# denix56/SI-Mamba

Hardware: AMD Instinct MI355X
Metric: point-clouds/sec (fwd+bwd) (higher is better)
Workload: dtype f32; 1 GPU; PointMamba classifier train step (FPS+kNN grouping, encoder, spectral SAST ordering, 12 Mamba blocks d=384 at L=1024, head, AdamW), 1024 pts -> 128 patches; global_batch=64, per_gpu_batch=64, npoints=1024, patches=128, mamba_seq_len=1024, parallelism=dp1, communicator_ranks=1, library_gemm=tuned solution table (si_mamba_amd/tuned/gemm_gfx950.csv)

## Files before the change

si_mamba_amd/csrc/mfma_device.h:

```cpp
#pragma once
#include <type_traits>

#include "common.h"

namespace simamba {

typedef float f32x16 __attribute__((ext_vector_type(16)));
typedef float f32x4 __attribute__((ext_vector_type(4)));
typedef unsigned u32x4 __attribute__((ext_vector_type(4)));
typedef __bf16 bf16x8 __attribute__((ext_vector_type(8)));

using rsrc_t = __amdgpu_buffer_rsrc_t;
constexpr unsigned kOob = 0xfffff000u;

__device__ __forceinline__ rsrc_t make_rsrc(const void* base, unsigned bytes) {
  return __builtin_amdgcn_make_buffer_rsrc(const_cast<void*>(base), 0, static_cast<int>(bytes), 0x00020000);
}
using bvec4_t = decltype(__builtin_amdgcn_raw_buffer_load_b128(make_rsrc(nullptr, 0u), 0u, 0u, 0));
template <typename V>
__device__ __forceinline__ V bload16(rsrc_t r, unsigned voff, unsigned soff) {
  return __builtin_bit_cast(V, __builtin_amdgcn_raw_buffer_load_b128(r, voff, soff, 0));
}
template <typename V>
__device__ __forceinline__ void bstore16(V v, rsrc_t r, unsigned voff, unsigned soff) {
  __builtin_amdgcn_raw_buffer_store_b128(__builtin_bit_cast(bvec4_t, v), r, voff, soff, 0);
}
__device__ __forceinline__ void bstore4(float f, rsrc_t r, unsigned voff, unsigned soff) {
  __builtin_amdgcn_raw_buffer_store_b32(__builtin_bit_cast(unsigned, f), r, voff, soff, 0);
}
__device__ __forceinline__ void bstore2(unsigned short v, rsrc_t r, unsigned voff, unsigned soff) {
  __builtin_amdgcn_raw_buffer_store_b16(v, r, voff, soff, 0);
}

template <int I, int N, typename F>
__device__ __forceinline__ void static_for(F&& f) {
  if constexpr (I < N) {
    f(std::integral_constant<int, I>{});
    static_for<I + 1, N>(f);
  }
}
template <int OFF, typename V>
__device__ __forceinline__ void lds_read16(V& dst, unsigned addr) {
  asm volatile("ds_read_b128 %0, %1 offset:%2" : "=v"(dst) : "v"(addr), "n"(OFF) : "memory");
}
template <int N, typename V>
__device__ __forceinline__ void lds_wait(V& v) {
  asm volatile("s_waitcnt lgkmcnt(%1)" : "+v"(v) : "n"(N) : "memory");
}

__device__ __forceinline__ unsigned bf16_pack2(float lo, float hi) {
  return static_cast<unsigned>(f32_to_bf16(lo)) | (static_cast<unsigned>(f32_to_bf16(hi)) << 16);
}
__device__ __forceinline__ float bf16_lo(unsigned w) { return __builtin_bit_cast(float, w << 16); }
__device__ __forceinline__ float bf16_hi(unsigned w) { return __builtin_bit_cast(float, w & 0xffff0000u); }

}
```

si_mamba_amd/csrc/scan_bwd_seq.hip:

```cpp
#include "scan_host.h"
#include "scan_seq_common.h"
#include "scan_xlane.h"

namespace simamba {

#ifndef SIMAMBA_BWDSEQ_OCC
#define SIMAMBA_BWDSEQ_OCC 3
#endif
constexpr int kBsSeg = 16;
constexpr int kBsR = 16;
constexpr int kBsWaves = 4;
constexpr int kBsThreads = 64 * kBsWaves;
constexpr int kBsCh = kBsR * kBsWaves;
constexpr int kBsTile = kBsR * kSeqTC;
constexpr int kBsPPitch = 33;
constexpr int kBsWaveFloats = 4 * kBsTile + kSeqTC * kBsPPitch;
constexpr int kBsSmemFloats = kBsWaves * kBsWaveFloats + kSeqTC * 32;

struct BwdSeqArgs {
  const void* u; const void* delta; const void* z; const void* dout;
  void* du; void* ddelta; void* dz;
  const float* A; const float* D; const float* delta_bias;
  const void* B; const void* C;
  const void* dt; const void* wdt;
  long long dt_bs, dt_ts;
  int dt_rank;
  const float* ckpt;
  float* dA; float* dB; float* dC; float* dD; float* ddelta_bias;
  int batch, dim, seqlen, nck;
  int bc_mode;
  long long z_bs, dz_bs;
  long long bc_bs, bc_ns, bc_ts;
};

__device__ __forceinline__ float bs_row_finish(float w0, float w1) {
  float d;
  asm("s_nop 1\n\t"
      "v_add_f32_dpp %0, %1, %1 row_ror:8 row_mask:0xf bank_mask:0x3\n\t"
      "v_add_f32_dpp %0, %2, %2 row_ror:8 row_mask:0xf bank_mask:0xc\n\t"
      "s_nop 1\n\t"
      "v_add_f32_dpp %0, %0, %0 row_shr:4 row_mask:0xf bank_mask:0xa"
      : "=&v"(d)
      : "v"(w0), "v"(w1));
  return d;
}

__device__ __forceinline__ void bs_quad_sum1(float& a) {
  asm("s_nop 1\n\t"
      "v_add_f32_dpp %0, %0, %0 quad_perm:[1,0,3,2] row_mask:0xf bank_mask:0xf\n\t"
      "s_nop 1\n\t"
      "v_add_f32_dpp %0, %0, %0 quad_perm:[2,3,0,1] row_mask:0xf bank_mask:0xf"
      : "+v"(a));
}
__device__ __forceinline__ void bs_quad_sum2(float& a, float& b) {
  asm("s_nop 1\n\t"
      "v_add_f32_dpp %0, %0, %0 quad_perm:[1,0,3,2] row_mask:0xf bank_mask:0xf\n\t"
      "v_add_f32_dpp %1, %1, %1 quad_perm:[1,0,3,2] row_mask:0xf bank_mask:0xf\n\t"
      "s_nop 0\n\t"
      "v_add_f32_dpp %0, %0, %0 quad_perm:[2,3,0,1] row_mask:0xf bank_mask:0xf\n\t"
      "v_add_f32_dpp %1, %1, %1 quad_perm:[2,3,0,1] row_mask:0xf bank_mask:0xf"
      : "+v"(a), "+v"(b));
}

template <typename T, bool kHasZ, bool kDt = false, bool kDet = false>
__global__ __launch_bounds__(kBsThreads, SIMAMBA_BWDSEQ_OCC) void scan_bwd_seq_kernel(BwdSeqArgs p) {
  __shared__ __attribute__((aligned(16))) float smem[kBsSmemFloats];
  const int tid = threadIdx.x;
  const int lane = tid & 63;
  const int wave = __builtin_amdgcn_readfirstlane(tid >> 6);
  int tile_id, b;
  xcd_tile(tile_id, b);
  const int L = p.seqlen, D = p.dim;
  const int d0w = tile_id * kBsCh + wave * kBsR;
  float* tD = smem + wave * kBsWaveFloats;
  float* tU = tD + kBsTile;
  float* tY = tU + kBsTile;
  float* tZ = tY + kBsTile;
  float* tP = tZ + kBsTile;
  float* tBC = smem + kBsWaves * kBsWaveFloats;

  const int r4 = lane >> 4, cq = (lane >> 2) & 3, pq = lane & 3;
  const int ch = 4 * r4 + cq;
  const int dch = d0w + ch;
  float A2[4];
  {
    const float4 a4 = *reinterpret_cast<const float4*>(p.A + static_cast<size_t>(dch) * kMaxState + 4 * pq);
    A2[0] = a4.x * kLog2e; A2[1] = a4.y * kLog2e; A2[2] = a4.z * kLog2e; A2[3] = a4.w * kLog2e;
  }
  const float Dfull = p.D ? p.D[dch] : 0.f;
  float ga[4] = {0.f, 0.f, 0.f, 0.f};
  float dAacc[4] = {0.f, 0.f, 0.f, 0.f};
  float dDacc = 0.f;
  const int sw = (ch >> 1) & 7;
  const int trow = ch * kSeqTC;
  const int pf = (r4 >> 1) * 16 + 4 * pq + 2 * (r4 & 1) + (cq >> 1);
  const float* ckl = p.ckpt + (static_cast<size_t>(b) * p.nck * D + dch) * kMaxState + 4 * pq;
  float* tDb = smem + wave * kBsWaveFloats + 4 * kBsTile + kSeqTC;
  if (kDet && lane < kBsR) tDb[lane * kBsPPitch] = 0.f;

  constexpr unsigned kEsz = sizeof(T);
  const unsigned zdelta = (static_cast<unsigned>(b * p.z_bs) - static_cast<unsigned>(b) * D * L) * kEsz;
  const unsigned dzdelta = (static_cast<unsigned>(b * p.dz_bs) - static_cast<unsigned>(b) * D * L) * kEsz;
  const T* __restrict__ ug = static_cast<const T*>(p.u);
  const T* __restrict__ dg = static_cast<const T*>(p.delta);
  const T* __restrict__ zg = static_cast<const T*>(p.z);
  const T* __restrict__ gg = static_cast<const T*>(p.dout);
  T* __restrict__ dug = static_cast<T*>(p.du);
  T* __restrict__ ddg = static_cast<T*>(p.ddelta);
  T* __restrict__ dzg = static_cast<T*>(p.dz);
  auto lane_now = [&]() -> int {
    int l = __builtin_amdgcn_mbcnt_hi(~0u, __builtin_amdgcn_mbcnt_lo(~0u, 0u));
    asm volatile("" : "+v"(l));
    return l;
  };
  auto row_off = [&](int l, int j) -> unsigned {
    return ((static_cast<unsigned>(b) * D + d0w + (l >> 3) + 8 * j) * L + 4 * (l & 7)) * kEsz;
  };

  const bool tok = p.bc_mode == 2;
  const T* __restrict__ Bgp = static_cast<const T*>(p.B) + static_cast<long long>(b) * p.bc_bs;
  const T* __restrict__ Cgp = static_cast<const T*>(p.C) + static_cast<long long>(b) * p.bc_bs;
  float bcv[4];
  auto issue_bc = [&](int t0, int tv) {
    const bool isC = tok ? (tv & 4) != 0 : (tv >> 7) != 0;
    const int bc_n = tok ? 4 * (tv & 3) : ((tv >> 3) & 15);
    const int bc_tl = tok ? (tv >> 3) : 4 * (tv & 7);
    const int t = (t0 + bc_tl < L) ? t0 + bc_tl : 0;
    const unsigned o = static_cast<unsigned>(bc_n * static_cast<int>(p.bc_ns) + t * static_cast<int>(p.bc_ts)) * kEsz;
    float vb[4], vc[4];
    if (isC) load4<T>(Cgp, o, vc); else load4<T>(Bgp, o, vb);
#pragma unroll
    for (int k = 0; k < 4; ++k) bcv[k] = isC ? vc[k] : vb[k];
  };
  auto stage_bc = [&](int tv) {
    if (tok) {
      *reinterpret_cast<float4*>(tBC + (tv >> 3) * 32 + 4 * (tv & 7)) = make_float4(bcv[0], bcv[1], bcv[2], bcv[3]);
    } else {
      float* dst = tBC + 4 * (tv & 7) * 32 + (tv >> 7) * 16 + ((tv >> 3) & 15);
#pragma unroll
      for (int k = 0; k < 4; ++k) dst[k * 32] = bcv[k];
    }
  };

  float dv[2][4], uv[2][4], gv[2][4], zv[2][4], hsn[4], biasA[2];
  auto form_delta = [&](int t0, int l) {
    const int mc = l & 15, mk = l >> 4;
    const T* wrow = static_cast<const T*>(p.wdt) + static_cast<size_t>(d0w + mc) * p.dt_rank;
    biasA[0] = p.delta_bias ? p.delta_bias[d0w + mc] : 0.f;
#pragma unroll
    for (int tile = 0; tile < 2; ++tile) {
      const int tt = t0 + 16 * tile + mc;
      const T* dtrow = static_cast<const T*>(p.dt) + static_cast<long long>(b) * p.dt_bs +
                       static_cast<long long>(tt < L ? tt : 0) * p.dt_ts;
      f32x4_t acc = {0.f, 0.f, 0.f, 0.f};
      if constexpr (sizeof(T) == 4) {
        const int c0 = (mk & 1) * 4 + (mk >> 1);
        float a[6], w[6];
#pragma unroll
        for (int m = 0; m < 6; ++m) {
          const int r = 8 * (m >> 1) + c0 + 2 * (m & 1);
          const int rc = min(r, p.dt_rank - 1);
          a[m] = reinterpret_cast<const float*>(dtrow)[rc];
          w[m] = reinterpret_cast<const float*>(wrow)[rc];
        }
#pragma unroll
        for (int m = 0; m < 6; ++m) {
          const int r = 8 * (m >> 1) + c0 + 2 * (m & 1);
          acc = __builtin_amdgcn_mfma_f32_16x16x4f32(r < p.dt_rank ? a[m] : 0.f, w[m], acc, 0, 0, 0);
        }
      } else {
        const int kc = min(8 * mk, p.dt_rank - 8);
        uint4 a8 = *reinterpret_cast<const uint4*>(reinterpret_cast<const uint16_t*>(dtrow) + kc);
        const uint4 w8 = *reinterpret_cast<const uint4*>(reinterpret_cast<const uint16_t*>(wrow) + kc);
        if (8 * mk >= p.dt_rank) a8 = make_uint4(0u, 0u, 0u, 0u);
        acc = __builtin_amdgcn_mfma_f32_16x16x32_bf16(__builtin_bit_cast(bf16x8, a8), __builtin_bit_cast(bf16x8, w8),
                                                      acc, 0, 0, 0);
#pragma unroll
        for (int e = 0; e < 4; ++e) acc[e] = bf16_to_f32(f32_to_bf16(acc[e]));
      }
#pragma unroll
      for (int e = 0; e < 4; ++e) dv[tile][e] = acc[e];
    }
  };
  auto load_state = [&](int ts) {
    float4 h4 = make_float4(0.f, 0.f, 0.f, 0.f);
    if (ts > 0 && ts < L) h4 = *reinterpret_cast<const float4*>(ckl + static_cast<size_t>(ts / kBsSeg - 1) * D * kMaxState);
    hsn[0] = h4.x; hsn[1] = h4.y; hsn[2] = h4.z; hsn[3] = h4.w;
  };
  auto issue_loads = [&](int t0, int l) {
    const int qv = l & 7;
    const bool in = t0 + 4 * qv < L;
    const unsigned to = in ? t0 * kEsz : 0u - 4u * qv * kEsz;
#pragma unroll
    for (int j = 0; j < 2; ++j) {
      const unsigned ro = row_off(l, j) + to;
      if (!kDt) load4<T>(dg, ro, dv[j]);
      load4<T>(ug, ro, uv[j]);
      load4<T>(gg, ro, gv[j]);
      if (kHasZ) load4<T>(zg, ro + zdelta, zv[j]);
      if (!kDt) biasA[j] = p.delta_bias ? p.delta_bias[d0w + (l >> 3) + 8 * j] : 0.f;
    }
    if (kDt) form_delta(t0, l);
    load_state(t0 + kBsSeg);
  };

  const int nchunks = (L + kSeqTC - 1) / kSeqTC;
  {
    const int t0 = (nchunks - 1) * kSeqTC;
    const int l = lane_now();
    issue_bc(t0, wave * 64 + l);
    issue_loads(t0, l);
    stage_bc(wave * 64 + l);
  }

  for (int c = nchunks - 1; c >= 0; --c) {
    const int t0 = c * kSeqTC;
    __syncthreads();

    {
      const int l = lane_now();
      const bool in_seq = t0 + 4 * (l & 7) < L;
      if (kDt) {
        const int mc = l & 15, mk = l >> 4;
#pragma unroll
        for (int tile = 0; tile < 2; ++tile) {
          const int qm = 4 * tile + mk;
          const float b2 = (t0 + 4 * qm < L) ? biasA[0] * kLog2e : -1e30f;
          float dl[4];
#pragma unroll
          for (int i = 0; i < 4; ++i) dl[i] = softplus_log2(fmaf(dv[tile][i], kLog2e, b2));
          *reinterpret_cast<float4*>(tD + tile_off(mc, qm)) = make_float4(dl[0], dl[1], dl[2], dl[3]);
        }
      }
#pragma unroll
      for (int j = 0; j < 2; ++j) {
        const float b2 = in_seq ? biasA[j] * kLog2e : -1e30f;
        float dl[4], dyv[4], dzw[4];
#pragma unroll
        for (int i = 0; i < 4; ++i) {
          if (!kDt) dl[i] = softplus_log2(fmaf(dv[j][i], kLog2e, b2));
          const float go = in_seq ? gv[j][i] : 0.f;
          if (kHasZ) {
            const float z = zv[j][i], sg = sigmoid_f(z);
            dyv[i] = go * z * sg;
            dzw[i] = go * sg * (1.f + z * (1.f - sg));
          } else {
            dyv[i] = go;
          }
        }
        const int to_ = tile_off((l >> 3) + 8 * j, l & 7);
        if (!kDt) *reinterpret_cast<float4*>(tD + to_) = make_float4(dl[0], dl[1], dl[2], dl[3]);
        *reinterpret_cast<float4*>(tU + to_) = make_float4(uv[j][0], uv[j][1], uv[j][2], uv[j][3]);
        *reinterpret_cast<float4*>(tY + to_) = make_float4(dyv[0], dyv[1], dyv[2], dyv[3]);
        if (kHasZ) *reinterpret_cast<float4*>(tZ + to_) = make_float4(dzw[0], dzw[1], dzw[2], dzw[3]);
      }
    }
    __builtin_amdgcn_fence(__ATOMIC_RELEASE, "wavefront");
    __builtin_amdgcn_wave_barrier();

#pragma unroll 1
    for (int seg = 1; seg >= 0; --seg) {
      const int ts = t0 + kBsSeg * seg;
      if (ts >= L) { load_state(t0); continue; }
      const float* bcp = tBC + seg * (kBsSeg * 32) + 4 * pq;
      const int gb = 4 * seg;

      float H[kBsSeg][4];
      {
        float h[4] = {hsn[0], hsn[1], hsn[2], hsn[3]};
        float d4[4], u4[4], z4[4];
#ifndef SIMAMBA_BWDSEQ_NOPREFETCH
        float4 b4n = *reinterpret_cast<const float4*>(bcp);
        float4 c4n = *reinterpret_cast<const float4*>(bcp + 16);
#endif
#pragma unroll
        for (int i = 0; i < kBsSeg; ++i) {
          const int o = trow + 4 * ((gb + (i >> 2)) ^ sw);
          if ((i & 3) == 0) {
            const float4 dd = *reinterpret_cast<const float4*>(tD + o);
            const float4 uu = *reinterpret_cast<const float4*>(tU + o);
            d4[0] = dd.x; d4[1] = dd.y; d4[2] = dd.z; d4[3] = dd.w;
            u4[0] = uu.x; u4[1] = uu.y; u4[2] = uu.z; u4[3] = uu.w;
            if (kHasZ) {
              const float4 zz = *reinterpret_cast<const float4*>(tZ + o);
              z4[0] = zz.x; z4[1] = zz.y; z4[2] = zz.z; z4[3] = zz.w;
            }
          }
#ifndef SIMAMBA_BWDSEQ_NOPREFETCH
          const float vB[4] = {b4n.x, b4n.y, b4n.z, b4n.w};
          const float vC[4] = {c4n.x, c4n.y, c4n.z, c4n.w};
          {
            const int in = (i + 1) & (kBsSeg - 1);
            b4n = *reinterpret_cast<const float4*>(bcp + in * 32);
            c4n = *reinterpret_cast<const float4*>(bcp + in * 32 + 16);
          }
          __builtin_amdgcn_sched_barrier(0);
#else
          const float4 b4 = *reinterpret_cast<const float4*>(bcp + i * 32);
          const float4 c4 = *reinterpret_cast<const float4*>(bcp + i * 32 + 16);
          const float vB[4] = {b4.x, b4.y, b4.z, b4.w};
          const float vC[4] = {c4.x, c4.y, c4.z, c4.w};
#endif
          const float dl = d4[i & 3], uu = u4[i & 3];
          const float xx = dl * uu;
          float y = 0.f;
#pragma unroll
          for (int j = 0; j < 4; ++j) {
            const float a = fast_exp2(dl * A2[j]);
            h[j] = fmaf(a, h[j], xx * vB[j]);
            H[i][j] = h[j];
            y = fmaf(vC[j], h[j], y);
          }
          if (kHasZ) {
            bs_quad_sum1(y);
            const float dzv = z4[i & 3] * fmaf(Dfull, uu, y);
            if (pq == 0) tZ[o + (i & 3)] = dzv;
          }
          __builtin_amdgcn_sched_barrier(0);
        }
      }

      {
        float d4[4], u4[4], y4[4];
        float hin[4] = {0.f, 0.f, 0.f, 0.f};
#ifndef SIMAMBA_BWDSEQ_NOPREFETCH
        float4 b4n = *reinterpret_cast<const float4*>(bcp + (kBsSeg - 1) * 32);
        float4 c4n = *reinterpret_cast<const float4*>(bcp + (kBsSeg - 1) * 32 + 16);
#endif
#pragma unroll
        for (int i = kBsSeg - 1; i >= 0; --i) {
          const int o = trow + 4 * ((gb + (i >> 2)) ^ sw);
          if ((i & 3) == 3) {
            const float4 dd = *reinterpret_cast<const float4*>(tD + o);
            const float4 uu = *reinterpret_cast<const float4*>(tU + o);
            const float4 yy = *reinterpret_cast<const float4*>(tY + o);
            d4[0] = dd.x; d4[1] = dd.y; d4[2] = dd.z; d4[3] = dd.w;
            u4[0] = uu.x; u4[1] = uu.y; u4[2] = uu.z; u4[3] = uu.w;
            y4[0] = yy.x; y4[1] = yy.y; y4[2] = yy.z; y4[3] = yy.w;
          }
          if (i == kBsSeg / 2 - 1) load_state(ts - kBsSeg);
          if (i == 1 && ts > 0) {
            const float4 h4 = *reinterpret_cast<const float4*>(ckl + static_cast<size_t>(ts / kBsSeg - 1) * D * kMaxState);
            hin[0] = h4.x; hin[1] = h4.y; hin[2] = h4.z; hin[3] = h4.w;
          }
#ifndef SIMAMBA_BWDSEQ_NOPREFETCH
          const float vB[4] = {b4n.x, b4n.y, b4n.z, b4n.w};
          const float vC[4] = {c4n.x, c4n.y, c4n.z, c4n.w};
          {
            const int in = (i + kBsSeg - 1) & (kBsSeg - 1);
            b4n = *reinterpret_cast<const float4*>(bcp + in * 32);
            c4n = *reinterpret_cast<const float4*>(bcp + in * 32 + 16);
          }
          __builtin_amdgcn_sched_barrier(0);
#else
          const float4 b4 = *reinterpret_cast<const float4*>(bcp + i * 32);
          const float4 c4 = *reinterpret_cast<const float4*>(bcp + i * 32 + 16);
          const float vB[4] = {b4.x, b4.y, b4.z, b4.w};
          const float vC[4] = {c4.x, c4.y, c4.z, c4.w};
#endif
          const float dl = d4[i & 3], uu = u4[i & 3], dy = y4[i & 3];
          const float xx = dl * uu;
          float dxs = 0.f, dda = 0.f;
          float red[8];
#pragma unroll
          for (int j = 0; j < 4; ++j) {
            const float g = fmaf(vC[j], dy, ga[j]);
            const float a = fast_exp2(dl * A2[j]);
            ga[j] = g * a;
            const float qv = ga[j] * ((i > 0) ? H[i > 0 ? i - 1 : 0][j] : hin[j]);
            dda = fmaf(A2[j], qv, dda);
            dAacc[j] = fmaf(dl, qv, dAacc[j]);
            dxs = fmaf(g, vB[j], dxs);
            red[j] = g * xx;
            red[4 + j] = dy * H[i][j];
          }
          bs_quad_sum2(dxs, dda);
          const float duv = fmaf(dl, dxs, Dfull * dy);
          const float t2v = fmaf(uu, dxs, kLn2 * dda);
          dDacc = fmaf(dy, uu, dDacc);
          if (pq == 0) {
            tU[o + (i & 3)] = duv;
            tY[o + (i & 3)] = t2v;
          }
#ifdef SIMAMBA_BWDSEQ_NORED
          const float s = red[0] + red[1] + red[2] + red[3] + red[4] + red[5] + red[6] + red[7];
#else
          swap32_stage<4>(red, red + 4);
          swap16_stage<2>(red, red + 2);
          const float s = bs_row_finish(red[0], red[1]);
#endif
          if ((cq & 1) == 1) tP[(kBsSeg * seg + i) * kBsPPitch + pf] = s;
          __builtin_amdgcn_sched_barrier(0);
        }
      }
    }
    __builtin_amdgcn_fence(__ATOMIC_RELEASE, "wavefront");
    __builtin_amdgcn_wave_barrier();

    {
      const int l = lane_now();
      const bool in_seq = t0 + 4 * (l & 7) < L;
#pragma unroll
      for (int j = 0; j < 2; ++j) {
        const int to_ = tile_off((l >> 3) + 8 * j, l & 7);
        const float4 a4 = *reinterpret_cast<const float4*>(tU + to_);
        const float4 t4 = *reinterpret_cast<const float4*>(tY + to_);
        const float4 d4 = *reinterpret_cast<const float4*>(tD + to_);
        const float duv[4] = {a4.x, a4.y, a4.z, a4.w};
        const float t2[4] = {t4.x, t4.y, t4.z, t4.w};
        const float dl[4] = {d4.x, d4.y, d4.z, d4.w};
        float dd[4], dsum = 0.f;
#pragma unroll
        for (int i = 0; i < 4; ++i) {
          dd[i] = t2[i] * softplus_grad_from_sp(dl[i]);
          dsum += dd[i];
        }
        const unsigned ro = row_off(l, j) + t0 * kEsz;
        if (in_seq) {
          store4<T>(dug, ro, duv);
          store4<T>(ddg, ro, dd);
          if (kHasZ) {
            const float4 z4 = *reinterpret_cast<const float4*>(tZ + to_);
            const float dzv[4] = {z4.x, z4.y, z4.z, z4.w};
            store4<T>(dzg, ro + dzdelta, dzv);
          }
        }
        if (p.ddelta_bias) {
          dsum += dpp<DPP_QUAD_XOR1>(0.f, dsum);
          dsum += dpp<DPP_QUAD_XOR2>(0.f, dsum);
          dsum += dpp<DPP_ROW_HALF_MIRROR>(0.f, dsum);
          if (kDet) {
            if ((l & 7) == 0) tDb[((l >> 3) + 8 * j) * kBsPPitch] += dsum;
          } else {
            if ((l & 7) == 0) atomicAdd(&p.ddelta_bias[d0w + (l >> 3) + 8 * j], dsum);
          }
        }
      }
      const int tn = c > 0 ? t0 - kSeqTC : 0;
      issue_loads(tn, l);
      issue_bc(tn, wave * 64 + l);
    }
    __syncthreads();

    {
      const int tv = wave * 64 + lane_now();
      stage_bc(tv);
#pragma unroll
      for (int k = 0; k < 4; ++k) {
        const int e = tv + kBsThreads * k;
        const int f = e >> 5, t = e & 31;
        float v = 0.f;
#pragma unroll
        for (int w = 0; w < kBsWaves; ++w) v += smem[w * kBsWaveFloats + 4 * kBsTile + t * kBsPPitch + f];
#ifdef SIMAMBA_BWDSEQ_NOFLUSH
        if (t0 + t < L && v == 123.456f) {
#else
        if (t0 + t < L) {
#endif
          if (kDet) {
            float* dst = ((f >> 4) ? p.dC : p.dB) + static_cast<size_t>(tile_id) * 2 * p.batch * kMaxState * L +
                         (static_cast<size_t>(b) * kMaxState + (f & 15)) * L + t0 + t;
            *dst = v;
          } else {
            float* dst = ((f >> 4) ? p.dC : p.dB) + (static_cast<size_t>(b) * kMaxState + (f & 15)) * L + t0 + t;
            atomicAdd(dst, v);
          }
        }
      }
    }
  }

  if (kDet) {
    const size_t row = static_cast<size_t>(b) * D + dch;
    *reinterpret_cast<float4*>(p.dA + row * kMaxState + 4 * pq) = make_float4(dAacc[0], dAacc[1], dAacc[2], dAacc[3]);
    if (p.dD && pq == 0) p.dD[row] = dDacc;
    const int l = lane_now();
    if (p.ddelta_bias && l < kBsR) p.ddelta_bias[static_cast<size_t>(b) * D + d0w + l] = tDb[l * kBsPPitch];
    return;
  }
#pragma unroll
  for (int j = 0; j < 4; ++j) atomicAdd(&p.dA[static_cast<size_t>(dch) * kMaxState + 4 * pq + j], dAacc[j]);
  if (p.dD && pq == 0) atomicAdd(&p.dD[dch], dDacc);
}

bool scan_bwd_seq_ok(int batch, int dim, int seqlen, int dstate, int softplus, int vec, long long z_bs, long long dz_bs,
                     bool has_z, int bc_mode, long long bc_ns, long long bc_ts) {
  const long long rows = static_cast<long long>(batch) * dim;
  return dstate == kMaxState && softplus && vec && dim % kBsCh == 0 && rows * seqlen < (1ll << 30) && bc_mode != 0 &&
         (!has_z || (static_cast<long long>(batch) * z_bs < (1ll << 30) &&
                     static_cast<long long>(batch) * dz_bs < (1ll << 30))) &&
         bc_ns >= 0 && bc_ts >= 0 && (kMaxState - 1) * bc_ns + (seqlen - 1) * bc_ts < (1ll << 30);
}

template <typename T, bool kDt, bool kDet>
static void launch_bwd_seq(const BwdSeqArgs& a, hipStream_t s) {
  dim3 grid(a.dim / kBsCh, a.batch);
  if constexpr (kDt)
    hipLaunchKernelGGL((scan_bwd_seq_kernel<T, true, true, kDet>), grid, dim3(kBsThreads), 0, s, a);
  else if (a.z)
    hipLaunchKernelGGL((scan_bwd_seq_kernel<T, true, false, kDet>), grid, dim3(kBsThreads), 0, s, a);
  else
    hipLaunchKernelGGL((scan_bwd_seq_kernel<T, false, false, kDet>), grid, dim3(kBsThreads), 0, s, a);
}
template <bool kDet>
static void launch_bwd_seq(const BwdSeqArgs& a, bool f32, hipStream_t s) {
  if (a.dt) { if (f32) launch_bwd_seq<float, true, kDet>(a, s); else launch_bwd_seq<bf16_t, true, kDet>(a, s); }
  else if (f32) launch_bwd_seq<float, false, kDet>(a, s); else launch_bwd_seq<bf16_t, false, kDet>(a, s);
}

int scan_bwd_seq_dispatch(const ScanArgs& sa, int io_dtype, int bc_mode, hipStream_t s, const void* dt, const void* wdt,
                          long long dt_bs, long long dt_ts, int dt_rank, bool det) {
  BwdSeqArgs a{};
  a.u = sa.u; a.delta = sa.delta; a.z = sa.z; a.dout = sa.dout;
  a.du = sa.du; a.ddelta = sa.ddelta; a.dz = sa.dz;
  a.A = sa.A; a.D = sa.D; a.delta_bias = sa.delta_bias; a.B = sa.B; a.C = sa.C;
  a.ckpt = sa.x_ckpt;
  a.dA = sa.dA; a.dB = sa.dB; a.dC = sa.dC; a.dD = sa.dD; a.ddelta_bias = sa.ddelta_bias;
  a.batch = sa.batch; a.dim = sa.dim; a.seqlen = sa.seqlen; a.nck = (sa.seqlen + kBsSeg - 1) / kBsSeg;
  a.bc_mode = bc_mode;
  a.z_bs = sa.z_bs; a.dz_bs = sa.dz_bs; a.bc_bs = sa.bc_bs; a.bc_ns = sa.bc_ns; a.bc_ts = sa.bc_ts;
  a.dt = dt; a.wdt = wdt; a.dt_bs = dt_bs; a.dt_ts = dt_ts; a.dt_rank = dt_rank;
  const bool f32 = io_dtype == SIMAMBA_F32;
  if (det) launch_bwd_seq<true>(a, f32, s); else launch_bwd_seq<false>(a, f32, s);
  return static_cast<int>(hipGetLastError());
}

}
```

Measured before the change: 1178 point-clouds/s.

## Use buffer resources for scan backward loads/stores and spread per-lane epilogue work

Replaces raw pointer arithmetic in the sequential backward scan with AMD buffer resource descriptors, using out-of-bounds offsets for masking instead of branches and clamped addresses. The per-step z/du/ddelta writes to LDS are redistributed so every lane in a quad writes one element instead of lane 0 writing all four. The row reduction for the state partial sums is split so pairs of steps are combined in one DPP step and written by all lanes. The dB/dC flush addressing is also simplified. The aim is to cut address VALU work, divergent stores and scalar bookkeeping in the main loop. The cost is extra registers for the resource descriptors and added reliance on hardware out-of-bounds behaviour.

```diff
diff --git a/si_mamba_amd/csrc/mfma_device.h b/si_mamba_amd/csrc/mfma_device.h
--- a/si_mamba_amd/csrc/mfma_device.h
+++ b/si_mamba_amd/csrc/mfma_device.h
@@ -24,6 +24,15 @@
 template <typename V>
 __device__ __forceinline__ void bstore16(V v, rsrc_t r, unsigned voff, unsigned soff) {
   __builtin_amdgcn_raw_buffer_store_b128(__builtin_bit_cast(bvec4_t, v), r, voff, soff, 0);
+}
+using bvec2_t = decltype(__builtin_amdgcn_raw_buffer_load_b64(make_rsrc(nullptr, 0u), 0u, 0u, 0));
+template <typename V>
+__device__ __forceinline__ V bload8(rsrc_t r, unsigned voff, unsigned soff) {
+  return __builtin_bit_cast(V, __builtin_amdgcn_raw_buffer_load_b64(r, voff, soff, 0));
+}
+template <typename V>
+__device__ __forceinline__ void bstore8(V v, rsrc_t r, unsigned voff, unsigned soff) {
+  __builtin_amdgcn_raw_buffer_store_b64(__builtin_bit_cast(bvec2_t, v), r, voff, soff, 0);
 }
 __device__ __forceinline__ void bstore4(float f, rsrc_t r, unsigned voff, unsigned soff) {
   __builtin_amdgcn_raw_buffer_store_b32(__builtin_bit_cast(unsigned, f), r, voff, soff, 0);
diff --git a/si_mamba_amd/csrc/scan_bwd_seq.hip b/si_mamba_amd/csrc/scan_bwd_seq.hip
--- a/si_mamba_amd/csrc/scan_bwd_seq.hip
+++ b/si_mamba_amd/csrc/scan_bwd_seq.hip
@@ -1,8 +1,26 @@
+#include "mfma_device.h"
 #include "scan_host.h"
 #include "scan_seq_common.h"
 #include "scan_xlane.h"
 
 namespace simamba {
+
+template <typename T>
+__device__ __forceinline__ void bload_pack(rsrc_t r, unsigned voff, unsigned soff, float (&v)[4]) {
+  Pack<T, 4> pk;
+  if constexpr (sizeof(T) == 4) pk = __builtin_bit_cast(Pack<T, 4>, bload16<float4>(r, voff, soff));
+  else pk = __builtin_bit_cast(Pack<T, 4>, bload8<uint2>(r, voff, soff));
+#pragma unroll
+  for (int i = 0; i < 4; ++i) v[i] = to_f32<T>(pk.v[i]);
+}
+template <typename T>
+__device__ __forceinline__ void bstore_pack(rsrc_t r, unsigned voff, unsigned soff, const float (&v)[4]) {
+  Pack<T, 4> pk;
+#pragma unroll
+  for (int i = 0; i < 4; ++i) pk.v[i] = from_f32<T>(v[i]);
+  if constexpr (sizeof(T) == 4) bstore16(__builtin_bit_cast(float4, pk), r, voff, soff);
+  else bstore8(__builtin_bit_cast(uint2, pk), r, voff, soff);
+}
 
 #ifndef SIMAMBA_BWDSEQ_OCC
 #define SIMAMBA_BWDSEQ_OCC 3
@@ -33,15 +51,22 @@
   long long bc_bs, bc_ns, bc_ts;
 };
 
-__device__ __forceinline__ float bs_row_finish(float w0, float w1) {
+__device__ __forceinline__ float bs_row_half(float w0, float w1) {
   float d;
   asm("s_nop 1\n\t"
       "v_add_f32_dpp %0, %1, %1 row_ror:8 row_mask:0xf bank_mask:0x3\n\t"
-      "v_add_f32_dpp %0, %2, %2 row_ror:8 row_mask:0xf bank_mask:0xc\n\t"
-      "s_nop 1\n\t"
-      "v_add_f32_dpp %0, %0, %0 row_shr:4 row_mask:0xf bank_mask:0xa"
+      "v_add_f32_dpp %0, %2, %2 row_ror:8 row_mask:0xf bank_mask:0xc"
       : "=&v"(d)
       : "v"(w0), "v"(w1));
+  return d;
+}
+__device__ __forceinline__ float bs_row_pair(float hi, float lo) {
+  float d;
+  asm("s_nop 1\n\t"
+      "v_add_f32_dpp %0, %1, %1 row_shr:4 row_mask:0xf bank_mask:0xa\n\t"
+      "v_add_f32_dpp %0, %2, %2 row_shl:4 row_mask:0xf bank_mask:0x5"
+      : "=&v"(d)
+      : "v"(hi), "v"(lo));
   return d;
 }
 
@@ -93,44 +118,54 @@
   float dDacc = 0.f;
   const int sw = (ch >> 1) & 7;
   const int trow = ch * kSeqTC;
-  const int pf = (r4 >> 1) * 16 + 4 * pq + 2 * (r4 & 1) + (cq >> 1);
-  const float* ckl = p.ckpt + (static_cast<size_t>(b) * p.nck * D + dch) * kMaxState + 4 * pq;
+  const int ppf = (r4 >> 1) * 16 + 4 * pq + 2 * (r4 & 1) + (cq >> 1) + (cq & 1) * kBsPPitch;
+  const rsrc_t rs_ck = make_rsrc(p.ckpt + (static_cast<size_t>(b) * p.nck * D + d0w) * kMaxState,
+                                 (static_cast<unsigned>(p.nck - 1) * D + kBsR) * kMaxState * 4u);
+  const unsigned ck_bs = static_cast<unsigned>(D) * kMaxState * 4u;
   float* tDb = smem + wave * kBsWaveFloats + 4 * kBsTile + kSeqTC;
   if (kDet && lane < kBsR) tDb[lane * kBsPPitch] = 0.f;
 
   constexpr unsigned kEsz = sizeof(T);
-  const unsigned zdelta = (static_cast<unsigned>(b * p.z_bs) - static_cast<unsigned>(b) * D * L) * kEsz;
-  const unsigned dzdelta = (static_cast<unsigned>(b * p.dz_bs) - static_cast<unsigned>(b) * D * L) * kEsz;
-  const T* __restrict__ ug = static_cast<const T*>(p.u);
-  const T* __restrict__ dg = static_cast<const T*>(p.delta);
-  const T* __restrict__ zg = static_cast<const T*>(p.z);
-  const T* __restrict__ gg = static_cast<const T*>(p.dout);
-  T* __restrict__ dug = static_cast<T*>(p.du);
-  T* __restrict__ ddg = static_cast<T*>(p.ddelta);
-  T* __restrict__ dzg = static_cast<T*>(p.dz);
+  const unsigned rowb = static_cast<unsigned>(L) * kEsz;
+  const size_t w0 = (static_cast<size_t>(b) * D + d0w) * L;
+  const size_t d0L = static_cast<size_t>(d0w) * L;
+  const rsrc_t rs_u = make_rsrc(static_cast<const T*>(p.u) + w0, kBsR * rowb);
+  const rsrc_t rs_d = make_rsrc(kDt ? nullptr : static_cast<const T*>(p.delta) + w0, kDt ? 0u : kBsR * rowb);
+  const rsrc_t rs_g = make_rsrc(static_cast<const T*>(p.dout) + w0, kBsR * rowb);
+  const rsrc_t rs_z = make_rsrc(kHasZ ? static_cast<const T*>(p.z) + b * p.z_bs + d0L : nullptr, kHasZ ? kBsR * rowb : 0u);
+  const rsrc_t rs_du = make_rsrc(static_cast<T*>(p.du) + w0, kBsR * rowb);
+  const rsrc_t rs_dd = make_rsrc(static_cast<T*>(p.ddelta) + w0, kBsR * rowb);
+  const rsrc_t rs_dz = make_rsrc(kHasZ ? static_cast<T*>(p.dz) + b * p.dz_bs + d0L : nullptr, kHasZ ? kBsR * rowb : 0u);
   auto lane_now = [&]() -> int {
-    int l = __builtin_amdgcn_mbcnt_hi(~0u, __builtin_amdgcn_mbcnt_lo(~0u, 0u));
-    asm volatile("" : "+v"(l));
-    return l;
-  };
-  auto row_off = [&](int l, int j) -> unsigned {
-    return ((static_cast<unsigned>(b) * D + d0w + (l >> 3) + 8 * j) * L + 4 * (l & 7)) * kEsz;
+    unsigned z = 0u;
+    asm volatile("" : "+v"(z));
+    return static_cast<int>(__builtin_amdgcn_mbcnt_hi(~0u, __builtin_amdgcn_mbcnt_lo(~0u, z)));
+  };
+  auto pack_off = [&](int l, int t0) -> unsigned {
+    const unsigned q = static_cast<unsigned>(l & 7);
+    const unsigned o = static_cast<unsigned>(l >> 3) * rowb + q * (4u * kEsz);
+    return t0 + 4 * static_cast<int>(q) < L ? o : kOob;
   };
 
   const bool tok = p.bc_mode == 2;
-  const T* __restrict__ Bgp = static_cast<const T*>(p.B) + static_cast<long long>(b) * p.bc_bs;
-  const T* __restrict__ Cgp = static_cast<const T*>(p.C) + static_cast<long long>(b) * p.bc_bs;
+  const unsigned bc_bytes =
+      static_cast<unsigned>((kMaxState - 1) * static_cast<int>(p.bc_ns) + (L - 1) * static_cast<int>(p.bc_ts) + 1) * kEsz;
+  const rsrc_t rs_B = make_rsrc(static_cast<const T*>(p.B) + static_cast<long long>(b) * p.bc_bs, bc_bytes);
+  const rsrc_t rs_C = make_rsrc(static_cast<const T*>(p.C) + static_cast<long long>(b) * p.bc_bs, bc_bytes);
   float bcv[4];
   auto issue_bc = [&](int t0, int tv) {
     const bool isC = tok ? (tv & 4) != 0 : (tv >> 7) != 0;
     const int bc_n = tok ? 4 * (tv & 3) : ((tv >> 3) & 15);
     const int bc_tl = tok ? (tv >> 3) : 4 * (tv & 7);
-    const int t = (t0 + bc_tl < L) ? t0 + bc_tl : 0;
-    const unsigned o = static_cast<unsigned>(bc_n * static_cast<int>(p.bc_ns) + t * static_cast<int>(p.bc_ts)) * kEsz;
+    const bool in = t0 + bc_tl < L;
+    const unsigned o = static_cast<unsigned>(bc_n * static_cast<int>(p.bc_ns) + bc_tl * static_cast<int>(p.bc_ts)) * kEsz;
+    const unsigned so = static_cast<unsigned>(t0 * static_cast<int>(p.bc_ts)) * kEsz;
     float vb[4], vc[4];
-    if (isC) load4<T>(Cgp, o, vc); else load4<T>(Bgp, o, vb);
-#pragma unroll
-    for (int k = 0; k < 4; ++k) bcv[k] = isC ? vc[k] : vb[k];
+    bload_pack<T>(rs_B, (in && !isC) ? o : kOob, so, vb);
+    bload_pack<T>(rs_C, (in && isC) ? o : kOob, so, vc);
+#pragma unroll
+    for (int k = 0; k < 4; ++k)
+      bcv[k] = __builtin_bit_cast(float, __builtin_bit_cast(unsigned, vb[k]) | __builtin_bit_cast(unsigned, vc[k]));
   };
   auto stage_bc = [&](int tv) {
     if (tok) {
@@ -184,20 +219,18 @@
   };
   auto load_state = [&](int ts) {
     float4 h4 = make_float4(0.f, 0.f, 0.f, 0.f);
-    if (ts > 0 && ts < L) h4 = *reinterpret_cast<const float4*>(ckl + static_cast<size_t>(ts / kBsSeg - 1) * D * kMaxState);
+    if (ts > 0 && ts < L) h4 = bload16<float4>(rs_ck, 16u * lane_now(), (ts / kBsSeg - 1) * ck_bs);
     hsn[0] = h4.x; hsn[1] = h4.y; hsn[2] = h4.z; hsn[3] = h4.w;
   };
   auto issue_loads = [&](int t0, int l) {
-    const int qv = l & 7;
-    const bool in = t0 + 4 * qv < L;
-    const unsigned to = in ? t0 * kEsz : 0u - 4u * qv * kEsz;
+    const unsigned vo = pack_off(l, t0);
 #pragma unroll
     for (int j = 0; j < 2; ++j) {
-      const unsigned ro = row_off(l, j) + to;
-      if (!kDt) load4<T>(dg, ro, dv[j]);
-      load4<T>(ug, ro, uv[j]);
-      load4<T>(gg, ro, gv[j]);
-      if (kHasZ) load4<T>(zg, ro + zdelta, zv[j]);
+      const unsigned so = static_cast<unsigned>(t0) * kEsz + j * (8u * rowb);
+      if (!kDt) bload_pack<T>(rs_d, vo, so, dv[j]);
+      bload_pack<T>(rs_u, vo, so, uv[j]);
+      bload_pack<T>(rs_g, vo, so, gv[j]);
+      if (kHasZ) bload_pack<T>(rs_z, vo, so, zv[j]);
       if (!kDt) biasA[j] = p.delta_bias ? p.delta_bias[d0w + (l >> 3) + 8 * j] : 0.f;
     }
     if (kDt) form_delta(t0, l);
@@ -268,7 +301,7 @@
       float H[kBsSeg][4];
       {
         float h[4] = {hsn[0], hsn[1], hsn[2], hsn[3]};
-        float d4[4], u4[4], z4[4];
+        float d4[4], u4[4], yk = 0.f, zo = 0.f, uo = 0.f;
 #ifndef SIMAMBA_BWDSEQ_NOPREFETCH
         float4 b4n = *reinterpret_cast<const float4*>(bcp);
         float4 c4n = *reinterpret_cast<const float4*>(bcp + 16);
@@ -281,11 +314,8 @@
             const float4 uu = *reinterpret_cast<const float4*>(tU + o);
             d4[0] = dd.x; d4[1] = dd.y; d4[2] = dd.z; d4[3] = dd.w;
             u4[0] = uu.x; u4[1] = uu.y; u4[2] = uu.z; u4[3] = uu.w;
-            if (kHasZ) {
-              const float4 zz = *reinterpret_cast<const float4*>(tZ + o);
-              z4[0] = zz.x; z4[1] = zz.y; z4[2] = zz.z; z4[3] = zz.w;
-            }
-          }
+          }
+          if (kHasZ && (i & 3) == 2) { zo = tZ[o + pq]; uo = tU[o + pq]; }
 #ifndef SIMAMBA_BWDSEQ_NOPREFETCH
           const float vB[4] = {b4n.x, b4n.y, b4n.z, b4n.w};
           const float vC[4] = {c4n.x, c4n.y, c4n.z, c4n.w};
@@ -313,15 +343,15 @@
           }
           if (kHasZ) {
             bs_quad_sum1(y);
-            const float dzv = z4[i & 3] * fmaf(Dfull, uu, y);
-            if (pq == 0) tZ[o + (i & 3)] = dzv;
+            yk = ((i & 3) == 0 || pq == (i & 3)) ? y : yk;
+            if ((i & 3) == 3) tZ[o + pq] = zo * fmaf(Dfull, uo, yk);
           }
           __builtin_amdgcn_sched_barrier(0);
         }
       }
 
       {
-        float d4[4], u4[4], y4[4];
+        float d4[4], u4[4], y4[4], xk = 0.f, ak = 0.f, sk = 0.f, dlo = 0.f, uo = 0.f, dyo = 0.f;
         float hin[4] = {0.f, 0.f, 0.f, 0.f};
 #ifndef SIMAMBA_BWDSEQ_NOPREFETCH
         float4 b4n = *reinterpret_cast<const float4*>(bcp + (kBsSeg - 1) * 32);
@@ -338,9 +368,10 @@
             u4[0] = uu.x; u4[1] = uu.y; u4[2] = uu.z; u4[3] = uu.w;
             y4[0] = yy.x; y4[1] = yy.y; y4[2] = yy.z; y4[3] = yy.w;
           }
+          if ((i & 3) == 1) { dlo = tD[o + pq]; uo = tU[o + pq]; dyo = tY[o + pq]; }
           if (i == kBsSeg / 2 - 1) load_state(ts - kBsSeg);
           if (i == 1 && ts > 0) {
-            const float4 h4 = *reinterpret_cast<const float4*>(ckl + static_cast<size_t>(ts / kBsSeg - 1) * D * kMaxState);
+            const float4 h4 = bload16<float4>(rs_ck, 16u * lane_now(), (ts / kBsSeg - 1) * ck_bs);
             hin[0] = h4.x; hin[1] = h4.y; hin[2] = h4.z; hin[3] = h4.w;
           }
 #ifndef SIMAMBA_BWDSEQ_NOPREFETCH
@@ -375,21 +406,22 @@
             red[4 + j] = dy * H[i][j];
           }
           bs_quad_sum2(dxs, dda);
-          const float duv = fmaf(dl, dxs, Dfull * dy);
-          const float t2v = fmaf(uu, dxs, kLn2 * dda);
           dDacc = fmaf(dy, uu, dDacc);
-          if (pq == 0) {
-            tU[o + (i & 3)] = duv;
-            tY[o + (i & 3)] = t2v;
+          xk = ((i & 3) == 3 || pq == (i & 3)) ? dxs : xk;
+          ak = ((i & 3) == 3 || pq == (i & 3)) ? dda : ak;
+          if ((i & 3) == 0) {
+            tU[o + pq] = fmaf(dlo, xk, Dfull * dyo);
+            tY[o + pq] = fmaf(uo, xk, kLn2 * ak);
           }
 #ifdef SIMAMBA_BWDSEQ_NORED
           const float s = red[0] + red[1] + red[2] + red[3] + red[4] + red[5] + red[6] + red[7];
 #else
           swap32_stage<4>(red, red + 4);
           swap16_stage<2>(red, red + 2);
-          const float s = bs_row_finish(red[0], red[1]);
-#endif
-          if ((cq & 1) == 1) tP[(kBsSeg * seg + i) * kBsPPitch + pf] = s;
+          const float s = bs_row_half(red[0], red[1]);
+#endif
+          if (i & 1) sk = s;
+          else tP[(kBsSeg * seg + i) * kBsPPitch + ppf] = bs_row_pair(sk, s);
           __builtin_amdgcn_sched_barrier(0);
         }
       }
@@ -399,7 +431,7 @@
 
     {
       const int l = lane_now();
-      const bool in_seq = t0 + 4 * (l & 7) < L;
+      const unsigned vo = pack_off(l, t0);
 #pragma unroll
       for (int j = 0; j < 2; ++j) {
         const int to_ = tile_off((l >> 3) + 8 * j, l & 7);
@@ -415,15 +447,13 @@
           dd[i] = t2[i] * softplus_grad_from_sp(dl[i]);
           dsum += dd[i];
         }
-        const unsigned ro = row_off(l, j) + t0 * kEsz;
-        if (in_seq) {
-          store4<T>(dug, ro, duv);
-          store4<T>(ddg, ro, dd);
-          if (kHasZ) {
-            const float4 z4 = *reinterpret_cast<const float4*>(tZ + to_);
-            const float dzv[4] = {z4.x, z4.y, z4.z, z4.w};
-            store4<T>(dzg, ro + dzdelta, dzv);
-          }
+        const unsigned so = static_cast<unsigned>(t0) * kEsz + j * (8u * rowb);
+        bstore_pack<T>(rs_du, vo, so, duv);
+        bstore_pack<T>(rs_dd, vo, so, dd);
+        if (kHasZ) {
+          const float4 z4 = *reinterpret_cast<const float4*>(tZ + to_);
+          const float dzv[4] = {z4.x, z4.y, z4.z, z4.w};
+          bstore_pack<T>(rs_dz, vo, so, dzv);
         }
         if (p.ddelta_bias) {
           dsum += dpp<DPP_QUAD_XOR1>(0.f, dsum);
@@ -445,42 +475,42 @@
     {
       const int tv = wave * 64 + lane_now();
       stage_bc(tv);
+      const int t = tv & 31, fr = tv >> 5;
+      const unsigned eo = static_cast<unsigned>(fr * L + t) * 4u;
+      const float* src = smem + 4 * kBsTile + t * kBsPPitch + fr;
+      const bool in = t0 + t < L;
 #pragma unroll
       for (int k = 0; k < 4; ++k) {
-        const int e = tv + kBsThreads * k;
-        const int f = e >> 5, t = e & 31;
         float v = 0.f;
 #pragma unroll
-        for (int w = 0; w < kBsWaves; ++w) v += smem[w * kBsWaveFloats + 4 * kBsTile + t * kBsPPitch + f];
+        for (int w = 0; w < kBsWaves; ++w) v += src[w * kBsWaveFloats + 8 * k];
+        float* base = ((k >> 1) ? p.dC : p.dB) + (static_cast<size_t>(b) * kMaxState + 8 * (k & 1)) * L + t0;
+        if (kDet) base += static_cast<size_t>(tile_id) * 2 * p.batch * kMaxState * L;
+        float* dst = reinterpret_cast<float*>(reinterpret_cast<char*>(base) + eo);
 #ifdef SIMAMBA_BWDSEQ_NOFLUSH
-        if (t0 + t < L && v == 123.456f) {
+        if (in && v == 123.456f) {
 #else
-        if (t0 + t < L) {
-#endif
-          if (kDet) {
-            float* dst = ((f >> 4) ? p.dC : p.dB) + static_cast<size_t>(tile_id) * 2 * p.batch * kMaxState * L +
-                         (static_cast<size_t>(b) * kMaxState + (f & 15)) * L + t0 + t;
-            *dst = v;
-          } else {
-            float* dst = ((f >> 4) ? p.dC : p.dB) + (static_cast<size_t>(b) * kMaxState + (f & 15)) * L + t0 + t;
-            atomicAdd(dst, v);
-          }
+        if (in) {
+#endif
+          if (kDet) *dst = v;
+          else atomicAdd(dst, v);
         }
       }
     }
   }
 
+  const int l = lane_now();
   if (kDet) {
-    const size_t row = static_cast<size_t>(b) * D + dch;
-    *reinterpret_cast<float4*>(p.dA + row * kMaxState + 4 * pq) = make_float4(dAacc[0], dAacc[1], dAacc[2], dAacc[3]);
-    if (p.dD && pq == 0) p.dD[row] = dDacc;
-    const int l = lane_now();
-    if (p.ddelta_bias && l < kBsR) p.ddelta_bias[static_cast<size_t>(b) * D + d0w + l] = tDb[l * kBsPPitch];
+    const size_t row0 = static_cast<size_t>(b) * D + d0w;
+    *reinterpret_cast<float4*>(p.dA + row0 * kMaxState + 4 * l) = make_float4(dAacc[0], dAacc[1], dAacc[2], dAacc[3]);
+    if (p.dD && (l & 3) == 0) p.dD[row0 + (l >> 2)] = dDacc;
+    if (p.ddelta_bias && l < kBsR) p.ddelta_bias[row0 + l] = tDb[l * kBsPPitch];
     return;
   }
-#pragma unroll
-  for (int j = 0; j < 4; ++j) atomicAdd(&p.dA[static_cast<size_t>(dch) * kMaxState + 4 * pq + j], dAacc[j]);
-  if (p.dD && pq == 0) atomicAdd(&p.dD[dch], dDacc);
+  float* dAw = p.dA + static_cast<size_t>(d0w) * kMaxState;
+#pragma unroll
+  for (int j = 0; j < 4; ++j) atomicAdd(&dAw[4 * l + j], dAacc[j]);
+  if (p.dD && (l & 3) == 0) atomicAdd(&p.dD[d0w + (l >> 2)], dDacc);
 }
 
 bool scan_bwd_seq_ok(int batch, int dim, int seqlen, int dstate, int softplus, int vec, long long z_bs, long long dz_bs,
```

Measured after the change: 1179 point-clouds/s (median of 2 runs). About the same (+0.1%).
